# matvogel/P2P-Bridge

Measured on AMD Instinct MI355X. Metric: denoised points/sec (8192-pt patches, T=30), higher is better.
Workload: dtype f32; 1 GPU; PVDS_PUNet xyz-only, 8192-pt patches, T=30 bridge steps, batch 32 per GPU (BASELINE configs[1]); patches_per_gpu=32, points_per_patch=8192, bridge_steps=30, parallelism=patch-shard x1, process_group_world_size=1, hipgraph=True, weights=seeded random init (26.44 M params)

## Files before the change

p2p_bridge_amd/csrc/conv3d_farfield.hip:

```cpp
#include "conv3d_common.h"

static __global__ void far_value_kernel(int c, const float *__restrict__ base, const float *__restrict__ scale,
                                 const float *__restrict__ shift, int swish, float *__restrict__ a) {
  const int b = blockIdx.y, ch = blockIdx.x * 256 + threadIdx.x;
  if (ch >= c) return;
  a[(size_t)b * c + ch] = xf_apply(base[ch], scale[(size_t)b * c + ch], shift[(size_t)b * c + ch], swish);
}

static __global__ __launch_bounds__(256) void tap_sum_kernel(int cin, int cout, int nchunk, int cout_pad,
                                                      const float *__restrict__ wt, const float *__restrict__ a,
                                                      float *__restrict__ tsum) {
  const int tap = blockIdx.y, b = blockIdx.z;
  const int co = blockIdx.x * 256 + threadIdx.x;
  if (co >= cout) return;
  float acc = 0.0f;
  for (int ci = 0; ci < cin; ++ci) {
    const size_t idx = ((((size_t)tap * nchunk + (ci >> 3)) * 2 + (ci & 1)) * cout_pad + co) * 4 + ((ci & 7) >> 1);
    acc = __fmaf_rn(wt[idx], a[(size_t)b * cin + ci], acc);
  }
  tsum[((size_t)b * 27 + tap) * cout + co] = acc;
}

static __global__ __launch_bounds__(256) void class_bias_kernel(int cout, const float *__restrict__ tsum,
                                                         const float *__restrict__ bias, float *__restrict__ k_out) {
  const int cls = blockIdx.y, b = blockIdx.z;
  const int co = blockIdx.x * 256 + threadIdx.x;
  if (co >= cout) return;
  const int cd = cls / 9, ch = (cls / 3) % 3, cw = cls % 3;
  float acc = 0.0f;
  for (int tap = 0; tap < 27; ++tap) {
    const int kd = tap / 9, kh = (tap / 3) % 3, kw = tap % 3;
    if ((cd == 0 && kd == 0) || (cd == 2 && kd == 2) || (ch == 0 && kh == 0) || (ch == 2 && kh == 2) ||
        (cw == 0 && kw == 0) || (cw == 2 && kw == 2))
      continue;
    acc += tsum[((size_t)b * 27 + tap) * cout + co];
  }
  k_out[((size_t)b * 27 + cls) * cout + co] = acc + bias[co];
}

constexpr int FF_CO = 32;
static __global__ __launch_bounds__(1024) void far_field_kernel(int cin, int cout, int nchunk, int cout_pad,
                                                        const float *__restrict__ base, const float *__restrict__ scale,
                                                        const float *__restrict__ shift, int swish,
                                                        const float *__restrict__ wt, const float *__restrict__ bias,
                                                        float *__restrict__ a_out, float *__restrict__ k_out,
                                                        const float *__restrict__ part, int nslots, GnFinish fin) {
  extern __shared__ double ff_sm_d[];
  float *ff_sm = (float *)ff_sm_d;
  const int b = blockIdx.y, t = threadIdx.x, c = t & (FF_CO - 1), tap = t / FF_CO;
  const int co = blockIdx.x * FF_CO + c;
  float *a, *T;
  if (part != nullptr) {
    float *tsc = ff_sm, *tsh = ff_sm + cin;
    double *gl = ff_sm_d + (2 * cin + 1) / 2;
    GnFinish f = fin;
    if (blockIdx.x != 0) f.scale = f.shift = nullptr;
    gn_finish_sample<4>(cin, nslots, part, f, b, gl, tsc, tsh);
    a = (float *)gl, T = a + nchunk * 8;
    for (int ch = t; ch < cin; ch += 1024) {
      const float v = xf_apply(base[ch], tsc[ch], tsh[ch], swish);
      a[ch] = v;
      if (blockIdx.x == 0) a_out[(size_t)b * cin + ch] = v;
    }
  } else {
    a = ff_sm, T = ff_sm + nchunk * 8;
    for (int ch = t; ch < cin; ch += 1024) {
      const float v = xf_apply(base[ch], scale[(size_t)b * cin + ch], shift[(size_t)b * cin + ch], swish);
      a[ch] = v;
      if (blockIdx.x == 0) a_out[(size_t)b * cin + ch] = v;
    }
  }
  __syncthreads();
  if (tap < 27) {
    float acc = 0.0f;
    if (co < cout) {
      const float4 *w4 = (const float4 *)wt + ((size_t)tap * nchunk * 2) * cout_pad + co;
#pragma unroll 4
      for (int k8 = 0; k8 < nchunk; ++k8) {
        const float4 h0 = w4[(size_t)(2 * k8) * cout_pad], h1 = w4[(size_t)(2 * k8 + 1) * cout_pad];
        const float *av = a + k8 * 8;
        const int left = cin - k8 * 8;
        if (left > 0) acc = __fmaf_rn(h0.x, av[0], acc);
        if (left > 1) acc = __fmaf_rn(h1.x, av[1], acc);
        if (left > 2) acc = __fmaf_rn(h0.y, av[2], acc);
        if (left > 3) acc = __fmaf_rn(h1.y, av[3], acc);
        if (left > 4) acc = __fmaf_rn(h0.z, av[4], acc);
        if (left > 5) acc = __fmaf_rn(h1.z, av[5], acc);
        if (left > 6) acc = __fmaf_rn(h0.w, av[6], acc);
        if (left > 7) acc = __fmaf_rn(h1.w, av[7], acc);
      }
    }
    T[tap * FF_CO + c] = acc;
  }
  __syncthreads();
  if (co >= cout || tap >= 27) return;
  {
    const int cls = tap;
    const int cd = cls / 9, ch = (cls / 3) % 3, cw = cls % 3;
    float acc = 0.0f;
    for (int tp = 0; tp < 27; ++tp) {
      const int kd = tp / 9, kh = (tp / 3) % 3, kw = tp % 3;
      if ((cd == 0 && kd == 0) || (cd == 2 && kd == 2) || (ch == 0 && kh == 0) || (ch == 2 && kh == 2) ||
          (cw == 0 && kw == 0) || (cw == 2 && kw == 2))
        continue;
      acc += T[tp * FF_CO + c];
    }
    k_out[((size_t)b * 27 + cls) * cout + co] = acc + bias[co];
  }
}

static int far_field_launch(int b, int cin, int cout, const float *prev_bias, const float *in_scale, const float *in_shift,
                            int in_swish, const float *wt_packed, const float *bias, float *a, float *k_out, float *tap_ws,
                            const float *part, int nslots, const GnFinish &fin, hipStream_t s) {
  const int nchunk = (cin + CONV_CK - 1) / CONV_CK, cout_pad = (cout + 63) / 64 * 64;
  const size_t body = (size_t)(nchunk * 8 + 27 * FF_CO) * 4;
  const size_t lds = part ? (size_t)((2 * cin + 1) / 2) * 8 + (body > 32768 ? body : 32768) : body;
  if (lds <= 48 * 1024) {
    hipLaunchKernelGGL(far_field_kernel, dim3(cdiv(cout, FF_CO), b), dim3(1024), lds, s, cin, cout, nchunk, cout_pad, prev_bias,
                       in_scale, in_shift, in_swish, wt_packed, bias, a, k_out, part, nslots, fin);
    return p2pb_launch_status();
  }
  if (part) {
    const int e = p2pb_gn_affine_launch(b, cin, nslots, part, fin, s);
    if (e != 0) return e;
    in_scale = fin.scale, in_shift = fin.shift;
  }
  hipLaunchKernelGGL(far_value_kernel, dim3(cdiv(cin, 256), b), dim3(256), 0, s, cin, prev_bias, in_scale, in_shift,
                     in_swish, a);
  hipLaunchKernelGGL(tap_sum_kernel, dim3(cdiv(cout, 256), 27, b), dim3(256), 0, s, cin, cout, nchunk, cout_pad,
                     wt_packed, a, tap_ws);
  hipLaunchKernelGGL(class_bias_kernel, dim3(cdiv(cout, 256), 27, b), dim3(256), 0, s, cout, tap_ws, bias, k_out);
// ... 23 lines not shown
```

p2p_bridge_amd/csrc/neighbors.hip:

```cpp
#include "common.h"

template <int UNROLL>
__global__ __launch_bounds__(256) void ball_query_kernel(int n, int m, float r2, int u,
                                                         const float *__restrict__ centers,
                                                         const float *__restrict__ points, int *__restrict__ idx) {
  const int b = blockIdx.y;
  const int lane = lane_id();
  const int j = blockIdx.x * 4 + (threadIdx.x >> 6);
  if (j >= m) return;
  const float *p = points + (size_t)b * 3 * n;
  const float *ce = centers + (size_t)b * 3 * m;
  int *o = idx + ((size_t)b * m + j) * u;
  const float cx = ce[j], cy = ce[j + m], cz = ce[j + 2 * m];
  int cnt = 0, first = 0;
  for (int base = 0; base < n && cnt < u; base += 64 * UNROLL) {
    float px[UNROLL], py[UNROLL], pz[UNROLL];
#pragma unroll
    for (int q = 0; q < UNROLL; ++q) {
      const int k = base + q * 64 + lane;
      const bool ok = k < n;
      px[q] = ok ? p[k] : 0.0f;
      py[q] = ok ? p[k + n] : 0.0f;
      pz[q] = ok ? p[k + 2 * n] : 0.0f;
    }
// ... 119 lines not shown
  const int c0 = blockIdx.y * CC, c1 = min(c0 + CC, ct);
  for (int l = c0; l < c1; ++l) {
    float v;
    if (l < 3) v = coords[((size_t)b * 3 + l) * n + id] - centers[((size_t)b * 3 + l) * m + j];
    else v = feat[((size_t)b * c + (l - 3)) * n + id];
    out[((size_t)b * ct + l) * mu + q] = v;
  }
}

extern "C" int p2pb_group_concat(int b, int c, int n, int m, int u, const float *coords, const float *centers,
                                 const float *feat, const int *idx, float *out, void *stream) {
  if (b <= 0 || c < 0 || n <= 0 || m <= 0 || u <= 0) return P2PB_EINVAL;
  constexpr int CC = 8;
  hipLaunchKernelGGL(group_concat_kernel<CC>, dim3(cdiv((long)m * u, 256), cdiv(3 + c, CC), b), dim3(256), 0,
                     (hipStream_t)stream, c, n, m, u, coords, centers, feat, idx, out);
  return p2pb_launch_status();
}

__global__ __launch_bounds__(256) void nb_transpose_kernel(int c, int n, const float *__restrict__ in,
                                                           float *__restrict__ out) {
  __shared__ float t[32][33];
  const int b = blockIdx.z, n0 = blockIdx.x * 32, c0 = blockIdx.y * 32;
  const int tx = threadIdx.x & 31, ty = threadIdx.x >> 5;
  const float *src = in + (size_t)b * c * n;
  float *dst = out + (size_t)b * c * n;
#pragma unroll
  for (int k = 0; k < 4; ++k) {
    const int cc = c0 + ty + 8 * k, nn = n0 + tx;
    t[ty + 8 * k][tx] = (cc < c && nn < n) ? src[(size_t)cc * n + nn] : 0.0f;
  }
  __syncthreads();
#pragma unroll
  for (int k = 0; k < 4; ++k) {
    const int nn = n0 + ty + 8 * k, cc = c0 + tx;
    if (cc < c && nn < n) dst[(size_t)nn * c + cc] = t[tx][ty + 8 * k];
  }
}

__global__ __launch_bounds__(256) void group_sub_kernel(int c, int n, int m, int u, int nslots,
                                                        const float *__restrict__ zt, const float *__restrict__ cxt,
                                                        const int *__restrict__ idx, float *__restrict__ out,
                                                        float *__restrict__ stats) {
  __shared__ float tile[64][65];
  const int b = blockIdx.z, p0 = blockIdx.x * 64, t = threadIdx.x;
  const int lane = t & 63, wave = t >> 6;
  const int mu = m * u;
  const int qmine = p0 + wave * 16 + (lane & 15);
  const int id_mine = qmine < mu ? idx[(size_t)b * mu + qmine] : -1;
  const int cpl = c <= 32 ? 32 : 64, pps = 64 / cpl;
  const int sub = lane / cpl, chl = lane % cpl;
  {
    const int c0 = blockIdx.y * cpl;
    const int ch = c0 + chl;
#pragma unroll 4
    for (int it = 0; it < 16 / pps; ++it) {
      const int pl = wave * 16 + it * pps + sub;
      const int id = __shfl(id_mine, it * pps + sub);
      float v = 0.0f;
      if (id >= 0 && ch < c) {
        v = zt[((size_t)b * n + id) * c + ch];
        if (cxt) v -= cxt[((size_t)b * m + (p0 + pl) / u) * c + ch];
      }
      tile[chl][pl] = v;
    }
    __syncthreads();
    const int pt = lane;
    const int per = cpl / 4;
#pragma unroll
    for (int k = 0; k < 16; ++k) {
      const int cr = wave + 4 * k;
      const float v = tile[cr & 63][pt];
      if (k < per && c0 + cr < c) {
        if (out && p0 + pt < mu) out[((size_t)b * c + c0 + cr) * mu + p0 + pt] = v;
        const float s1 = halfwave_sum_to_last(v), s2 = halfwave_sum_to_last(v * v);
        if ((lane & 31) == 31) {
          float *p = stats + (((size_t)b * nslots + blockIdx.x * 2 + (lane >> 5)) * c + c0 + cr) * 2;
          p[0] = s1;
          p[1] = s2;
        }
      }
    }
    __syncthreads();
  }
}

#define GST_PW 128
template <int CPL>
__global__ __launch_bounds__(256) void group_stats_kernel(int c, int n, int m, int u, int nslots, const float *__restrict__ zt,
                                                          const float *__restrict__ cxt, const int *__restrict__ idx,
                                                          float *__restrict__ stats) {
  constexpr int PPS = 64 / CPL;
  const int b = blockIdx.z, lane = threadIdx.x & 63, wave = threadIdx.x >> 6;
  const int slot = blockIdx.x * 4 + wave;
  if (slot >= nslots) return;
  const int mu = m * u, p0 = slot * GST_PW;
  const int sub = lane / CPL, ch = blockIdx.y * CPL + lane % CPL;
  const int ia = p0 + lane < mu ? idx[(size_t)b * mu + p0 + lane] : -1;
  const int ib = p0 + 64 + lane < mu ? idx[(size_t)b * mu + p0 + 64 + lane] : -1;
  const float *zb = zt + (size_t)b * n * c + ch;
  const float *cb = cxt ? cxt + (size_t)b * m * c + ch : nullptr;
  float s1 = 0.0f, s2 = 0.0f;
  const bool chok = ch < c;
#pragma unroll 8
  for (int it = 0; it < GST_PW / PPS; ++it) {
    const int pl = it * PPS + sub;
    const int id = pl < 64 ? __shfl(ia, pl) : __shfl(ib, pl - 64);
    if (id >= 0 && chok) {
      float v = zb[(size_t)id * c];
      if (cb) v -= cb[(size_t)((p0 + pl) / u) * c];
      s1 += v;
      s2 += v * v;
    }
  }
  if (PPS == 2) {
    s1 += __shfl_xor(s1, 32);
    s2 += __shfl_xor(s2, 32);
  }
  if (chok && sub == 0) {
    float *q = stats + (((size_t)b * nslots + slot) * c + ch) * 2;
    q[0] = s1;
    q[1] = s2;
  }
}

extern "C" int p2pb_group_sub_stats_slots(int m, int u) { return (int)(((long)m * u + GST_PW - 1) / GST_PW); }
extern "C" int p2pb_group_sub_stats(int b, int c, int n, int m, int u, const float *zt, const float *cxt, const int *idx,
                                    float *stats_part, void *stream) {
  if (b <= 0 || c <= 0 || n <= 0 || m <= 0 || u <= 0 || !zt || !idx || !stats_part || (long)m * u > 0x7fffffffL) return P2PB_EINVAL;
  const int nslots = p2pb_group_sub_stats_slots(m, u);
  hipStream_t s = (hipStream_t)stream;
  if (c <= 32)
    hipLaunchKernelGGL(group_stats_kernel<32>, dim3(cdiv(nslots, 4), cdiv(c, 32), b), dim3(256), 0, s, c, n, m, u, nslots, zt, cxt, idx,
                       stats_part);
  else
    hipLaunchKernelGGL(group_stats_kernel<64>, dim3(cdiv(nslots, 4), cdiv(c, 64), b), dim3(256), 0, s, c, n, m, u, nslots, zt, cxt, idx,
                       stats_part);
  return p2pb_launch_status();
}

extern "C" size_t p2pb_group_sub_stats_floats(int b, int c, int m, int u) {
  return (size_t)b * (((size_t)m * u + 63) / 64 * 2) * c * 2;
}

extern "C" int p2pb_group_sub(int b, int c, int n, int m, int u, const float *z, const float *cx, const int *idx,
                              float *out, float *stats_part, float *ws, void *stream) {
  if (b <= 0 || c <= 0 || n <= 0 || m <= 0 || u <= 0 || !stats_part) return P2PB_EINVAL;
  hipStream_t s = (hipStream_t)stream;
  const float *zt = z, *cxt = cx;
  if (ws) {
    float *zw = ws, *cw = ws + (size_t)b * n * c;
    hipLaunchKernelGGL(nb_transpose_kernel, dim3(cdiv(n, 32), cdiv(c, 32), b), dim3(256), 0, s, c, n, z, zw);
    if (cx) hipLaunchKernelGGL(nb_transpose_kernel, dim3(cdiv(m, 32), cdiv(c, 32), b), dim3(256), 0, s, c, m, cx, cw);
    zt = zw;
    cxt = cx ? cw : nullptr;
  }
  const int nblk = (int)(((long)m * u + 63) / 64);
  hipLaunchKernelGGL(group_sub_kernel, dim3(nblk, cdiv(c, c <= 32 ? 32 : 64), b), dim3(256), 0, s, c, n, m, u, nblk * 2,
                     zt, cxt, idx, out, stats_part);
  return p2pb_launch_status();
}

__global__ __launch_bounds__(256) void gather_kernel(int c, int n, int m, const float *__restrict__ feat,
                                                     const int *__restrict__ idx, float *__restrict__ out) {
  const int b = blockIdx.z, l = blockIdx.y;
  const int j = blockIdx.x * 256 + threadIdx.x;
  if (j >= m) return;
  out[((size_t)b * c + l) * m + j] = feat[((size_t)b * c + l) * n + idx[(size_t)b * m + j]];
}

extern "C" int p2pb_gather_features_forward(int b, int c, int n, int m, const float *feat, const int *idx, float *out,
                                            void *stream) {
  if (b <= 0 || c <= 0 || n <= 0 || m <= 0) return P2PB_EINVAL;
  hipLaunchKernelGGL(gather_kernel, dim3(cdiv(m, 256), c, b), dim3(256), 0, (hipStream_t)stream, c, n, m, feat, idx,
                     out);
  return p2pb_launch_status();
}

#define NN_TILE 2048
__global__ __launch_bounds__(256) void three_nn_kernel(int n, int m, const float *__restrict__ points,
                                                       const float *__restrict__ centers, float *__restrict__ weights,
                                                       int *__restrict__ indices) {
  __shared__ float sc[3][NN_TILE];
  const int b = blockIdx.y;
  const int j = blockIdx.x * 256 + threadIdx.x;
  const float *p = points + (size_t)b * 3 * n;
  const float *ce = centers + (size_t)b * 3 * m;
  const bool ok = j < n;
  const float ux = ok ? p[j] : 0.0f, uy = ok ? p[j + n] : 0.0f, uz = ok ? p[j + 2 * n] : 0.0f;
  float best0 = INFINITY, best1 = INFINITY, best2 = INFINITY;
// ... 292 lines not shown
                                                 float *out, void *stream) {
  if (b <= 0 || c <= 0 || n <= 0 || m <= 0) return P2PB_EINVAL;
  hipStream_t s = (hipStream_t)stream;
  hipLaunchKernelGGL(three_nn_kernel, dim3(cdiv(n, 256), b), dim3(256), 0, s, n, m, points, centers, w, idx);
  constexpr int CC = 16;
  hipLaunchKernelGGL(three_interp_kernel<CC>, dim3(cdiv(n, 256), cdiv(c, CC), b), dim3(256), 0, s, c, m, n, cfeat,
                     idx, w, out);
  return p2pb_launch_status();
}

extern "C" int p2pb_three_nn(int b, int m, int n, const float *points, const float *centers, int *idx, float *w,
                             void *stream) {
  if (b <= 0 || n <= 0 || m <= 0) return P2PB_EINVAL;
  hipLaunchKernelGGL(three_nn_kernel, dim3(cdiv(n, 256), b), dim3(256), 0, (hipStream_t)stream, n, m, points, centers,
                     w, idx);
  return p2pb_launch_status();
}

extern "C" int p2pb_three_interpolate(int b, int c, int m, int n, const float *cfeat, const int *idx, const float *w,
                                      float *out, void *stream) {
  if (b <= 0 || c <= 0 || n <= 0 || m <= 0) return P2PB_EINVAL;
  constexpr int CC = 16;
  hipLaunchKernelGGL(three_interp_kernel<CC>, dim3(cdiv(n, 256), cdiv(c, CC), b), dim3(256), 0, (hipStream_t)stream, c,
                     m, n, cfeat, idx, w, out);
  return p2pb_launch_status();
}

__global__ __launch_bounds__(256) void three_interp_add_kernel(int c, int m, int n, int nslots,
                                                               const float *__restrict__ czt,
                                                               const int *__restrict__ indices,
                                                               const float *__restrict__ weights,
                                                               const float *__restrict__ add,
                                                               const float *__restrict__ bias, float *__restrict__ out,
                                                               float *__restrict__ stats) {
  __shared__ float tile[64][65];
  __shared__ int sid[64][3];
  __shared__ float sw[64][3];
  const int b = blockIdx.z, p0 = blockIdx.x * 64, t = threadIdx.x;
  const int lane = t & 63, wave = t >> 6;
  if (t < 64) {
    const int j = min(p0 + t, n - 1);
#pragma unroll
    for (int k = 0; k < 3; ++k) {
      sid[t][k] = indices[((size_t)b * 3 + k) * n + j];
      sw[t][k] = weights[((size_t)b * 3 + k) * n + j];
    }
  }
  __syncthreads();
  {
    const int c0 = blockIdx.y * 64;
    const int ch = c0 + lane;
    if (ch < c) {
      const float *f = czt + (size_t)b * m * c + ch;
#pragma unroll 4
      for (int pl = wave * 16; pl < wave * 16 + 16; ++pl)
        tile[lane][pl] = __fmaf_rn(f[(size_t)sid[pl][2] * c], sw[pl][2],
                                   __fmaf_rn(f[(size_t)sid[pl][1] * c], sw[pl][1], f[(size_t)sid[pl][0] * c] * sw[pl][0]));
    }
    __syncthreads();
    const int pt = lane;
    const bool pok = p0 + pt < n;
#pragma unroll
    for (int k = 0; k < 16; ++k) {
      const int cr = wave + 4 * k;
      if (c0 + cr < c) {
        float v = 0.0f;
        if (pok) {
          const size_t o = ((size_t)b * c + c0 + cr) * n + p0 + pt;
          v = tile[cr][pt];
          if (add) v += add[o];
          if (bias) v += bias[c0 + cr];
          out[o] = v;
        }
        const float s1 = halfwave_sum_to_last(v), s2 = halfwave_sum_to_last(v * v);
        if ((lane & 31) == 31) {
          float *p = stats + (((size_t)b * nslots + blockIdx.x * 2 + (lane >> 5)) * c + c0 + cr) * 2;
          p[0] = s1;
          p[1] = s2;
        }
      }
    }
    __syncthreads();
  }
}

extern "C" int p2pb_three_interpolate_add(int b, int c, int m, int n, const float *cz, const int *idx, const float *w,
                                          const float *add, const float *bias, float *out, float *stats_part,
                                          float *ws, void *stream) {
  if (b <= 0 || c <= 0 || n <= 0 || m <= 0 || !stats_part) return P2PB_EINVAL;
  hipStream_t s = (hipStream_t)stream;
  const float *czt = cz;
  if (ws) {
    hipLaunchKernelGGL(nb_transpose_kernel, dim3(cdiv(m, 32), cdiv(c, 32), b), dim3(256), 0, s, c, m, cz, ws);
    czt = ws;
  }
  const int nblk = (n + 63) / 64;
  hipLaunchKernelGGL(three_interp_add_kernel, dim3(nblk, cdiv(c, 64), b), dim3(256), 0, s, c, m, n, nblk * 2, czt, idx, w,
                     add, bias, out, stats_part);
  return p2pb_launch_status();
}
```

p2p_bridge_amd/csrc/pvconv_finish.hip:

```cpp
#include "common.h"

static __global__ __launch_bounds__(256) void gn_affine_kernel(int c, int groups, int nslots, double count_per_channel,
                                                        const float *__restrict__ part, const float *__restrict__ gamma,
                                                        const float *__restrict__ beta, const float *__restrict__ style,
                                                        int style_stride, float eps, float *__restrict__ scale,
                                                        float *__restrict__ shift, float *__restrict__ chmean,
                                                        float *__restrict__ mean_rstd) {
  __shared__ double lds[4 * 256];
  GnFinish f;
  f.gamma = gamma, f.beta = beta, f.style = style, f.scale = scale, f.shift = shift, f.chmean = chmean;
  f.count_per_channel = count_per_channel, f.style_stride = style_stride, f.groups = groups, f.eps = eps;
  gn_finish_group(c, nslots, part, f, blockIdx.y, blockIdx.x, lds, mean_rstd);
}

int p2pb_gn_affine_launch(int b, int c, int nslots, const float *part, const GnFinish &f, hipStream_t s) {
  hipLaunchKernelGGL(gn_affine_kernel, dim3(f.groups, b), dim3(256), 0, s, c, f.groups, nslots, f.count_per_channel, part, f.gamma,
                     f.beta, f.style, f.style_stride, f.eps, f.scale, f.shift, f.chmean, (float *)nullptr);
  return p2pb_launch_status();
}
extern "C" int p2pb_gn_affine_params_ex(int b, int c, int groups, int nslots, double count_per_channel,
                                        const float *part, const float *gamma, const float *beta, const float *style,
                                        int style_stride, float eps, float *scale, float *shift, float *chmean,
                                        float *mean_rstd, void *stream) {
  if (b <= 0 || c <= 0 || nslots <= 0 || !gn_shape_ok(c, groups, style, style_stride)) return P2PB_EINVAL;
  hipLaunchKernelGGL(gn_affine_kernel, dim3(groups, b), dim3(256), 0, (hipStream_t)stream, c, groups, nslots,
                     count_per_channel, part, gamma, beta, style, style_stride, eps, scale, shift, chmean, mean_rstd);
  return p2pb_launch_status();
}

extern "C" int p2pb_gn_affine_params(int b, int c, int groups, int nslots, double count_per_channel,
                                     const float *part, const float *gamma, const float *beta, const float *style,
                                     int style_stride, float eps, float *scale, float *shift, float *chmean,
                                     void *stream) {
  return p2pb_gn_affine_params_ex(b, c, groups, nslots, count_per_channel, part, gamma, beta, style, style_stride, eps,
                                  scale, shift, chmean, nullptr, stream);
}

__device__ __forceinline__ void se_hidden(int c, int hidden, const float *__restrict__ w1, const float *mean, float *hid) {
  const int lane = threadIdx.x & 63, wave = threadIdx.x >> 6, nw = blockDim.x >> 6;
  for (int h = wave; h < hidden; h += nw) {
    float acc = 0.0f;
    for (int i = lane; i < c; i += 64) acc = __fmaf_rn(w1[(size_t)h * c + i], mean[i], acc);
#pragma unroll
    for (int d = 32; d >= 1; d >>= 1) acc += __shfl_xor(acc, d);
    if (lane == 0) hid[h] = fmaxf(acc, 0.0f);
  }
}


static __global__ __launch_bounds__(256) void se_gate_affine_kernel(int c, int hidden, const float *__restrict__ chmean,
                                                             const float *__restrict__ w1, const float *__restrict__ w2,
                                                             const float *__restrict__ scale,
                                                             const float *__restrict__ shift, float *__restrict__ aff_a,
                                                             float *__restrict__ aff_b) {
  extern __shared__ float se_sm[];
  float *mean = se_sm, *hid = se_sm + c;
  const int b = blockIdx.x, t = threadIdx.x;
  for (int i = t; i < c; i += 256) mean[i] = chmean[(size_t)b * c + i];
  __syncthreads();
  se_hidden(c, hidden, w1, mean, hid);
  __syncthreads();
  for (int i = t; i < c; i += 256) {
    float acc = 0.0f;
    for (int h = 0; h < hidden; ++h) acc = __fmaf_rn(w2[(size_t)i * hidden + h], hid[h], acc);
    const float gate = 1.0f / (1.0f + expf(-acc));
    aff_a[(size_t)b * c + i] = scale[(size_t)b * c + i] * gate;
    aff_b[(size_t)b * c + i] = shift[(size_t)b * c + i] * gate;
  }
}

static __global__ __launch_bounds__(1024) void pvconv_tail_kernel(int c, int hidden, const float *__restrict__ part2, int nslots2,
                                                           GnFinish f2, const float *__restrict__ w1, const float *__restrict__ w2,
                                                           float *__restrict__ aff_a, float *__restrict__ aff_b,
                                                           int cp, const float *__restrict__ partp, int nslotsp, GnFinish fp) {
  extern __shared__ double pt_sm[];
  const int b = blockIdx.y, t = threadIdx.x;
  if (blockIdx.x == 1) {
    gn_finish_sample<4>(cp, nslotsp, partp, fp, b, pt_sm);
    return;
  }
  float *sc = (float *)(pt_sm + 4096), *sh = sc + c, *mean = sh + c, *hid = mean + c;
  gn_finish_sample<4>(c, nslots2, part2, f2, b, pt_sm, sc, sh, mean);
  if (hidden <= 0) {
    for (int i = t; i < c; i += 1024) {
      aff_a[(size_t)b * c + i] = sc[i];
      aff_b[(size_t)b * c + i] = sh[i];
    }
    return;
  }
  se_hidden(c, hidden, w1, mean, hid);
  __syncthreads();
  for (int i = t; i < c; i += 1024) {
    float acc = 0.0f;
    for (int h = 0; h < hidden; ++h) acc = __fmaf_rn(w2[(size_t)i * hidden + h], hid[h], acc);
    const float gate = 1.0f / (1.0f + expf(-acc));
// ... 34 lines not shown
```

p2p_bridge_amd/csrc/voxelize.hip:

```cpp
#include "common.h"

__global__ __launch_bounds__(1024) void voxel_coords_kernel(int n, int r, int normalize, float eps,
                                                            const float *__restrict__ coords,
                                                            float *__restrict__ norm, int *__restrict__ vox) {
  __shared__ double part[3][256];
  __shared__ float smax[1024];
  const int t = threadIdx.x;
  const float *c = coords + (size_t)blockIdx.x * 3 * n;
  float *o = norm + (size_t)blockIdx.x * 3 * n;
  int *v = vox + (size_t)blockIdx.x * 3 * n;
  if (t < 256) {
    double s0 = 0.0, s1 = 0.0, s2 = 0.0;
    for (int k0 = t; k0 < n; k0 += 8 * 256) {
      float x0[8], x1[8], x2[8];
#pragma unroll
      for (int u = 0; u < 8; ++u) {
        const int k = k0 + u * 256;
        const bool ok = k < n;
        x0[u] = ok ? c[k] : 0.0f;
        x1[u] = ok ? c[n + k] : 0.0f;
        x2[u] = ok ? c[2 * n + k] : 0.0f;
      }
#pragma unroll
      for (int u = 0; u < 8; ++u)
// ... 287 lines not shown
#pragma unroll
        for (int i = 0; i < 4; ++i)
          if (i < nch) acc[i] += fq[i] * div;
      }
    }
  }
  float *o = out + ((size_t)b * r3 + v) * c + ch;
  if (ALIGNED) {
    *(vox_f32x4 *)o = vox_f32x4{acc[0], acc[1], acc[2], acc[3]};
  } else {
#pragma unroll
    for (int i = 0; i < 4; ++i)
      if (i < nch) o[i] = acc[i];
  }
}

__global__ __launch_bounds__(256) void vox_gather_cl_occ_kernel(int c, int n, int r3, const int *__restrict__ cnt,
                                                                const int *__restrict__ cur,
                                                                const int *__restrict__ occ,
                                                                const int *__restrict__ nocc,
                                                                const int *__restrict__ slist,
                                                                const float *__restrict__ feat_t,
                                                                float *__restrict__ out) {
  const int b = blockIdx.y;
  const size_t total = (size_t)nocc[b] * c;
  for (size_t e = (size_t)blockIdx.x * 256 + threadIdx.x; e < total; e += (size_t)gridDim.x * 256) {
    const int k = (int)(e / c), ch = (int)(e % c);
    const int v = occ[(size_t)b * n + k];
    const int cn = cnt[(size_t)b * r3 + v];
    const int *seg = slist + (size_t)b * n + (cur[(size_t)b * r3 + v] - cn);
    const float div = (float)(1.0 / (double)(float)cn);
    const float *f = feat_t + (size_t)b * n * c + ch;
    float acc = 0.0f;
    for (int q = 0; q < cn; ++q) acc += f[(size_t)seg[q] * c] * div;
    out[((size_t)b * r3 + v) * c + ch] = acc;
  }
}

template <bool ALIGNED>
__global__ __launch_bounds__(256) void vox_gather_cl_split_kernel(int c, int nchunk, int n, int r3,
                                                                  const int *__restrict__ cnt, const int *__restrict__ cur,
                                                                  const int *__restrict__ slist,
                                                                  const float *__restrict__ feat_t, u32x4 *__restrict__ out) {
  const int b = blockIdx.y, ng = nchunk * 2;
  const size_t e = (size_t)blockIdx.x * 256 + threadIdx.x;
  if (e >= (size_t)r3 * ng) return;
  const int v = (int)(e / ng), g = (int)(e % ng), ch = g * 8;
  const int cn = cnt[(size_t)b * r3 + v];
  float acc[8] = {0.0f, 0.0f, 0.0f, 0.0f, 0.0f, 0.0f, 0.0f, 0.0f};
  if (cn > 0 && ch < c) {
    const int *seg = slist + (size_t)b * n + (cur[(size_t)b * r3 + v] - cn);
    const float div = (float)(1.0 / (double)(float)cn);
    const float *f = feat_t + (size_t)b * n * c + ch;
    for (int q = 0; q < cn; ++q) {
      const float *fq = f + (size_t)seg[q] * c;
      if (ALIGNED) {
#pragma unroll
        for (int h = 0; h < 2; ++h)
          if (ch + 4 * h < c) {
            const vox_f32x4 x = *(const vox_f32x4 *)(fq + 4 * h);
#pragma unroll
            for (int i = 0; i < 4; ++i) acc[4 * h + i] += x[i] * div;
          }
      } else {
#pragma unroll
        for (int i = 0; i < 8; ++i)
          if (ch + i < c) acc[i] += fq[i] * div;
      }
    }
  }
  u32x4 p0, p1;
#pragma unroll
  for (int i = 0; i < 4; ++i) {
    unsigned a0, a1, a2;
    split_pair<SPLIT_F16X3>(acc[2 * i], acc[2 * i + 1], a0, a1, a2);
    p0[i] = a0;
    p1[i] = a1;
  }
  u32x4 *dst = out + (((size_t)b * r3 + v) * nchunk + (g >> 1)) * 4 + (g & 1);
  dst[0] = p0;
  dst[2] = p1;
}

template <bool ALIGNED>
__global__ __launch_bounds__(256) void vox_gather_cl_occ_split_kernel(int c, int nchunk, int n, int r3,
                                                                      const int *__restrict__ cnt, const int *__restrict__ cur,
                                                                      const int *__restrict__ occ, const int *__restrict__ nocc,
                                                                      const int *__restrict__ slist,
                                                                      const float *__restrict__ feat_t, u32x4 *__restrict__ out) {
  const int b = blockIdx.y, ng = nchunk * 2;
  const size_t total = (size_t)nocc[b] * ng;
  for (size_t e = (size_t)blockIdx.x * 256 + threadIdx.x; e < total; e += (size_t)gridDim.x * 256) {
    const int k = (int)(e / ng), g = (int)(e % ng), ch = g * 8;
    const int v = occ[(size_t)b * n + k];
    const int cn = cnt[(size_t)b * r3 + v];
    const int *seg = slist + (size_t)b * n + (cur[(size_t)b * r3 + v] - cn);
    const float div = (float)(1.0 / (double)(float)cn);
    const float *f = feat_t + (size_t)b * n * c + ch;
    float acc[8] = {0.0f, 0.0f, 0.0f, 0.0f, 0.0f, 0.0f, 0.0f, 0.0f};
    for (int q0 = 0; q0 < cn; q0 += 4) {
      int id[4];
#pragma unroll
      for (int u = 0; u < 4; ++u) id[u] = seg[min(q0 + u, cn - 1)];
      float x[4][8];
#pragma unroll
      for (int u = 0; u < 4; ++u) {
        const float *fq = f + (size_t)id[u] * c;
        if (ALIGNED) {
#pragma unroll
          for (int h = 0; h < 2; ++h) {
            vox_f32x4 y = vox_f32x4{0.0f, 0.0f, 0.0f, 0.0f};
            if (ch + 4 * h < c) y = *(const vox_f32x4 *)(fq + 4 * h);
#pragma unroll
            for (int i = 0; i < 4; ++i) x[u][4 * h + i] = y[i];
          }
        } else {
#pragma unroll
          for (int i = 0; i < 8; ++i) x[u][i] = ch + i < c ? fq[i] : 0.0f;
        }
      }
#pragma unroll
// ... 206 lines not shown
extern "C" int p2pb_trilinear_devoxelize_forward(int b, int c, int n, int r, int is_training, const float *coords,
                                                 const float *feat, int *inds, float *wgts, float *outs,
                                                 void *stream) {
  if (b <= 0 || c <= 0 || n <= 0 || r <= 0) return P2PB_EINVAL;
  if (is_training && (!inds || !wgts)) return P2PB_EINVAL;
  constexpr int CC = 16;
  hipLaunchKernelGGL((devox_kernel<CC, false>), dim3(cdiv(n, 256), cdiv(c, CC), b), dim3(256), 0, (hipStream_t)stream,
                     c, n, r, is_training, coords, feat, (const float *)nullptr, (const float *)nullptr, inds, wgts,
                     outs);
  return p2pb_launch_status();
}

extern "C" int p2pb_trilinear_devoxelize_affine(int b, int c, int n, int r, const float *coords, const float *feat,
                                                const float *aff_a, const float *aff_b, float *outs, void *stream) {
  if (b <= 0 || c <= 0 || n <= 0 || r <= 0 || !aff_a || !aff_b) return P2PB_EINVAL;
  constexpr int CC = 16;
  hipLaunchKernelGGL((devox_kernel<CC, true>), dim3(cdiv(n, 256), cdiv(c, CC), b), dim3(256), 0, (hipStream_t)stream,
                     c, n, r, 0, coords, feat, aff_a, aff_b, (int *)nullptr, (float *)nullptr, outs);
  return p2pb_launch_status();
}

__global__ __launch_bounds__(256) void devox_cl_kernel(int c, int n, int r, const float *__restrict__ coords,
                                                       const float *__restrict__ grid, const float *__restrict__ aff_a,
                                                       const float *__restrict__ aff_b, const float *__restrict__ add,
                                                       const float *__restrict__ add_scale,
                                                       const float *__restrict__ add_shift, float *__restrict__ outs) {
  __shared__ float tile[64][65];
  __shared__ __attribute__((aligned(16))) int sidx[64][8];
  __shared__ __attribute__((aligned(16))) float sw[64][8];
  const int b = blockIdx.z, p0 = blockIdx.x * 64, t = threadIdx.x;
  const int lane = t & 63, wave = t >> 6;
  const int r3 = r * r * r;
  if (lane < 16) {
    const int tt = wave * 16 + lane;
    const int i = min(p0 + tt, n - 1);
    const float *co = coords + (size_t)b * 3 * n;
    const Corners k = devox_corners(co[i], co[i + n], co[i + 2 * n], r);
    typedef int i32x4 __attribute__((ext_vector_type(4)));
    typedef float f32x4 __attribute__((ext_vector_type(4)));
#define DV_LDS __attribute__((address_space(3)))
    *(volatile DV_LDS i32x4 *)&sidx[tt][0] = i32x4{k.idx[0], k.idx[1], k.idx[2], k.idx[3]};
    *(volatile DV_LDS i32x4 *)&sidx[tt][4] = i32x4{k.idx[4], k.idx[5], k.idx[6], k.idx[7]};
    *(volatile DV_LDS f32x4 *)&sw[tt][0] = f32x4{k.w[0], k.w[1], k.w[2], k.w[3]};
    *(volatile DV_LDS f32x4 *)&sw[tt][4] = f32x4{k.w[4], k.w[5], k.w[6], k.w[7]};
#undef DV_LDS
  }
  __syncthreads();
  const float *g = grid + (size_t)b * r3 * c;
  {
    const int c0 = blockIdx.y * 64;
    const int ch = c0 + lane;
    if (ch < c) {
      const float a = aff_a ? aff_a[(size_t)b * c + ch] : 1.0f, bb = aff_b ? aff_b[(size_t)b * c + ch] : 0.0f;
#pragma unroll 2
      for (int pl = wave * 16; pl < wave * 16 + 16; ++pl) {
        float fv[8];
#pragma unroll
        for (int q = 0; q < 8; ++q) fv[q] = g[(size_t)sidx[pl][q] * c + ch];
        if (aff_a) {
#pragma unroll
          for (int q = 0; q < 8; ++q) fv[q] = fv[q] * a + bb;
        }
        float acc = sw[pl][0] * fv[0];
#pragma unroll
        for (int q = 1; q < 8; ++q) acc = __fmaf_rn(sw[pl][q], fv[q], acc);
        tile[lane][pl] = acc;
      }
    }
    __syncthreads();
    const int pt = t & 63;
    if (p0 + pt < n) {
#pragma unroll
      for (int k = 0; k < 16; ++k) {
        const int cr = (t >> 6) + 4 * k;
        if (c0 + cr < c) {
          const size_t o = ((size_t)b * c + c0 + cr) * n + p0 + pt;
          float v = tile[cr][pt];
          if (add) {
            const float z = add[o] * add_scale[(size_t)b * c + c0 + cr] + add_shift[(size_t)b * c + c0 + cr];
            v = z * __builtin_amdgcn_rcpf(1.0f + __builtin_amdgcn_exp2f(z * -1.44269504088896340736f)) + v;
          }
          outs[o] = v;
        }
      }
    }
    __syncthreads();
  }
}

__global__ __launch_bounds__(256) void devox_cl4_kernel(int c, int n, int r, const float *__restrict__ coords,
                                                        const float *__restrict__ grid, const float *__restrict__ aff_a,
                                                        const float *__restrict__ aff_b, const float *__restrict__ add,
                                                        const float *__restrict__ add_scale,
                                                        const float *__restrict__ add_shift, float *__restrict__ outs) {
  __shared__ float tile[64][65];
  __shared__ __attribute__((aligned(16))) int sidx[64][8];
  __shared__ __attribute__((aligned(16))) float sw[64][8];
  typedef int i32x4 __attribute__((ext_vector_type(4)));
  typedef float f32x4 __attribute__((ext_vector_type(4)));
  const int b = blockIdx.z, p0 = blockIdx.x * 64, t = threadIdx.x;
  const int lane = t & 63, wave = t >> 6;
  const int r3 = r * r * r;
  if (lane < 16) {
    const int tt = wave * 16 + lane;
    const int i = min(p0 + tt, n - 1);
    const float *co = coords + (size_t)b * 3 * n;
    const Corners k = devox_corners(co[i], co[i + n], co[i + 2 * n], r);
#define DV_LDS __attribute__((address_space(3)))
    *(volatile DV_LDS i32x4 *)&sidx[tt][0] = i32x4{k.idx[0], k.idx[1], k.idx[2], k.idx[3]};
    *(volatile DV_LDS i32x4 *)&sidx[tt][4] = i32x4{k.idx[4], k.idx[5], k.idx[6], k.idx[7]};
    *(volatile DV_LDS f32x4 *)&sw[tt][0] = f32x4{k.w[0], k.w[1], k.w[2], k.w[3]};
    *(volatile DV_LDS f32x4 *)&sw[tt][4] = f32x4{k.w[4], k.w[5], k.w[6], k.w[7]};
#undef DV_LDS
  }
  __syncthreads();
  const float *g = grid + (size_t)b * r3 * c;
  const int c0 = blockIdx.y * 64;
  {
    const int cq = lane & 15, ps = lane >> 4;
    const int ch4 = c0 + 4 * cq;
    f32x4 a4 = {1.0f, 1.0f, 1.0f, 1.0f}, b4 = {0.0f, 0.0f, 0.0f, 0.0f};
    if (aff_a) {
      a4 = *(const f32x4 *)(aff_a + (size_t)b * c + ch4);
      b4 = *(const f32x4 *)(aff_b + (size_t)b * c + ch4);
    }
#pragma unroll 2
    for (int it = 0; it < 4; ++it) {
      const int pl = wave * 16 + it * 4 + ps;
      f32x4 fv[8];
#pragma unroll
      for (int q = 0; q < 8; ++q) fv[q] = *(const f32x4 *)(g + (size_t)sidx[pl][q] * c + ch4);
      if (aff_a) {
#pragma unroll
        for (int q = 0; q < 8; ++q)
#pragma unroll
          for (int i = 0; i < 4; ++i) fv[q][i] = fv[q][i] * a4[i] + b4[i];
      }
#pragma unroll
      for (int i = 0; i < 4; ++i) {
        float acc = sw[pl][0] * fv[0][i];
#pragma unroll
        for (int q = 1; q < 8; ++q) acc = __fmaf_rn(sw[pl][q], fv[q][i], acc);
        tile[4 * cq + i][pl] = acc;
      }
    }
  }
  __syncthreads();
  const int pt = t & 63;
  if (p0 + pt < n) {
#pragma unroll
    for (int k = 0; k < 16; ++k) {
      const int cr = (t >> 6) + 4 * k;
      const size_t o = ((size_t)b * c + c0 + cr) * n + p0 + pt;
      float v = tile[cr][pt];
      if (add) {
        const float z = add[o] * add_scale[(size_t)b * c + c0 + cr] + add_shift[(size_t)b * c + c0 + cr];
        v = z * __builtin_amdgcn_rcpf(1.0f + __builtin_amdgcn_exp2f(z * -1.44269504088896340736f)) + v;
      }
      outs[o] = v;
    }
  }
}

extern "C" int p2pb_trilinear_devoxelize_cl_affine(int b, int c, int n, int r, const float *coords, const float *grid,
                                                   const float *aff_a, const float *aff_b, const float *add,
                                                   const float *add_scale, const float *add_shift, float *outs,
                                                   void *stream) {
  if (b <= 0 || c <= 0 || n <= 0 || r <= 0 || ((aff_a == nullptr) != (aff_b == nullptr))) return P2PB_EINVAL;
  if (add && (!add_scale || !add_shift)) return P2PB_EINVAL;
  static const long wide = p2pb_experiment_long("devox_cl4", 1);
  if (wide && c % 64 == 0 && (((size_t)grid | (size_t)aff_a | (size_t)aff_b) & 15) == 0)
    hipLaunchKernelGGL(devox_cl4_kernel, dim3(cdiv(n, 64), c / 64, b), dim3(256), 0, (hipStream_t)stream, c, n, r, coords, grid,
                       aff_a, aff_b, add, add_scale, add_shift, outs);
  else
    hipLaunchKernelGGL(devox_cl_kernel, dim3(cdiv(n, 64), cdiv(c, 64), b), dim3(256), 0, (hipStream_t)stream, c, n, r, coords, grid,
                       aff_a, aff_b, add, add_scale, add_shift, outs);
  return p2pb_launch_status();
}
```

Baseline: 1.197 million points/s.

## Batch independent gather loads ahead of use across several memory-bound kernels

Several gather and reduction loops (far-field tap sums, group gather and group stats, the SE hidden matvec, voxel averaging, and trilinear devoxelization) are rewritten to issue a batch of independent global loads into registers before consuming them, using clamped indices and selects instead of guarded loads. Epilogue operands (residual add, scale and shift, bias) are prefetched before the barrier so their latency overlaps with the tile computation. Group stats also gains a compile-time flag for the centroid-subtract path. The aim is more memory-level parallelism in latency-bound gathers, paid for with higher register pressure, possible occupancy loss, and redundant clamped loads for out-of-range elements.

```diff
diff --git a/p2p_bridge_amd/csrc/conv3d_farfield.hip b/p2p_bridge_amd/csrc/conv3d_farfield.hip
--- a/p2p_bridge_amd/csrc/conv3d_farfield.hip
+++ b/p2p_bridge_amd/csrc/conv3d_farfield.hip
@@ -75,8 +75,26 @@
     float acc = 0.0f;
     if (co < cout) {
       const float4 *w4 = (const float4 *)wt + ((size_t)tap * nchunk * 2) * cout_pad + co;
-#pragma unroll 4
-      for (int k8 = 0; k8 < nchunk; ++k8) {
+      int k8 = 0;
+      for (; k8 + 4 <= cin / 8; k8 += 4) {
+        float4 h[8];
+#pragma unroll
+        for (int q = 0; q < 8; ++q) h[q] = w4[(size_t)(2 * k8 + q) * cout_pad];
+#pragma unroll
+        for (int q = 0; q < 4; ++q) {
+          const float4 h0 = h[2 * q], h1 = h[2 * q + 1];
+          const float *av = a + (k8 + q) * 8;
+          acc = __fmaf_rn(h0.x, av[0], acc);
+          acc = __fmaf_rn(h1.x, av[1], acc);
+          acc = __fmaf_rn(h0.y, av[2], acc);
+          acc = __fmaf_rn(h1.y, av[3], acc);
+          acc = __fmaf_rn(h0.z, av[4], acc);
+          acc = __fmaf_rn(h1.z, av[5], acc);
+          acc = __fmaf_rn(h0.w, av[6], acc);
+          acc = __fmaf_rn(h1.w, av[7], acc);
+        }
+      }
+      for (; k8 < nchunk; ++k8) {
         const float4 h0 = w4[(size_t)(2 * k8) * cout_pad], h1 = w4[(size_t)(2 * k8 + 1) * cout_pad];
         const float *av = a + k8 * 8;
         const int left = cin - k8 * 8;
diff --git a/p2p_bridge_amd/csrc/neighbors.hip b/p2p_bridge_amd/csrc/neighbors.hip
--- a/p2p_bridge_amd/csrc/neighbors.hip
+++ b/p2p_bridge_amd/csrc/neighbors.hip
@@ -195,16 +195,31 @@
   {
     const int c0 = blockIdx.y * cpl;
     const int ch = c0 + chl;
-#pragma unroll 4
-    for (int it = 0; it < 16 / pps; ++it) {
-      const int pl = wave * 16 + it * pps + sub;
-      const int id = __shfl(id_mine, it * pps + sub);
-      float v = 0.0f;
-      if (id >= 0 && ch < c) {
-        v = zt[((size_t)b * n + id) * c + ch];
-        if (cxt) v -= cxt[((size_t)b * m + (p0 + pl) / u) * c + ch];
-      }
-      tile[chl][pl] = v;
+    const float *zb = zt + (size_t)b * n * c + min(ch, c - 1);
+    const float *cb = cxt ? cxt + (size_t)b * m * c + min(ch, c - 1) : nullptr;
+    int cj = (p0 + wave * 16 + sub) / u, cr = (p0 + wave * 16 + sub) - cj * u;
+    for (int it0 = 0; it0 < 16 / pps; it0 += 8) {
+      int id[8];
+      float zv[8], cv[8];
+#pragma unroll
+      for (int k = 0; k < 8; ++k) {
+        id[k] = __shfl(id_mine, (it0 + k) * pps + sub);
+        zv[k] = zb[(size_t)max(id[k], 0) * c];
+        cv[k] = cb ? cb[(size_t)min(cj, m - 1) * c] : 0.0f;
+#pragma unroll
+        for (int q = 0; q < 2; ++q) {
+          const bool wrap = q < pps && cr + 1 == u;
+          cr = wrap ? 0 : (q < pps ? cr + 1 : cr);
+          cj += wrap ? 1 : 0;
+        }
+      }
+#pragma unroll
+      for (int k = 0; k < 8; ++k) {
+        const int pl = wave * 16 + (it0 + k) * pps + sub;
+        float v = zv[k];
+        if (cb) v -= cv[k];
+        tile[chl][pl] = (id[k] >= 0 && ch < c) ? v : 0.0f;
+      }
     }
     __syncthreads();
     const int pt = lane;
@@ -228,7 +243,8 @@
 }
 
 #define GST_PW 128
-template <int CPL>
+#define GST_NB 16
+template <int CPL, bool CX>
 __global__ __launch_bounds__(256) void group_stats_kernel(int c, int n, int m, int u, int nslots, const float *__restrict__ zt,
                                                           const float *__restrict__ cxt, const int *__restrict__ idx,
                                                           float *__restrict__ stats) {
@@ -240,19 +256,40 @@
   const int sub = lane / CPL, ch = blockIdx.y * CPL + lane % CPL;
   const int ia = p0 + lane < mu ? idx[(size_t)b * mu + p0 + lane] : -1;
   const int ib = p0 + 64 + lane < mu ? idx[(size_t)b * mu + p0 + 64 + lane] : -1;
-  const float *zb = zt + (size_t)b * n * c + ch;
-  const float *cb = cxt ? cxt + (size_t)b * m * c + ch : nullptr;
+  const bool chok = ch < c;
+  const float *zb = zt + (size_t)b * n * c + min(ch, c - 1);
+  const float *cb = CX ? cxt + (size_t)b * m * c + min(ch, c - 1) : nullptr;
+  int cj = (p0 + sub) / u, cr = (p0 + sub) - cj * u;
   float s1 = 0.0f, s2 = 0.0f;
-  const bool chok = ch < c;
-#pragma unroll 8
-  for (int it = 0; it < GST_PW / PPS; ++it) {
-    const int pl = it * PPS + sub;
-    const int id = pl < 64 ? __shfl(ia, pl) : __shfl(ib, pl - 64);
-    if (id >= 0 && chok) {
-      float v = zb[(size_t)id * c];
-      if (cb) v -= cb[(size_t)((p0 + pl) / u) * c];
-      s1 += v;
-      s2 += v * v;
+#pragma unroll 1
+  for (int pb = 0; pb < GST_PW; pb += GST_NB * PPS) {
+    const int src = pb < 64 ? ia : ib;
+    int id[GST_NB];
+    float zv[GST_NB], cv[GST_NB];
+#pragma unroll
+    for (int k = 0; k < GST_NB; ++k) {
+      const int l = (pb & 63) + k * PPS;
+      id[k] = __builtin_amdgcn_readlane(src, l);
+      if (PPS == 2) id[k] = sub ? __builtin_amdgcn_readlane(src, l + 1) : id[k];
+      zv[k] = zb[(size_t)max(id[k], 0) * c];
+      if (CX) {
+        cv[k] = cb[(size_t)min(cj, m - 1) * c];
+#pragma unroll
+        for (int q = 0; q < PPS; ++q) {
+          const bool wrap = cr + 1 == u;
+          cr = wrap ? 0 : cr + 1;
+          cj += wrap ? 1 : 0;
+        }
+      }
+    }
+#pragma unroll
+    for (int k = 0; k < GST_NB; ++k) {
+      float v = zv[k];
+      if (CX) v -= cv[k];
+      const bool ok = id[k] >= 0 && chok;
+      const float t1 = s1 + v, t2 = s2 + v * v;
+      s1 = ok ? t1 : s1;
+      s2 = ok ? t2 : s2;
     }
   }
   if (PPS == 2) {
@@ -264,6 +301,14 @@
     q[0] = s1;
     q[1] = s2;
   }
+}
+
+template <int CPL>
+static void group_stats_launch(int b, int c, int n, int m, int u, int nslots, const float *zt, const float *cxt, const int *idx,
+                               float *stats_part, hipStream_t s) {
+  const dim3 grid(cdiv(nslots, 4), cdiv(c, CPL), b);
+  if (cxt) hipLaunchKernelGGL((group_stats_kernel<CPL, true>), grid, dim3(256), 0, s, c, n, m, u, nslots, zt, cxt, idx, stats_part);
+  else hipLaunchKernelGGL((group_stats_kernel<CPL, false>), grid, dim3(256), 0, s, c, n, m, u, nslots, zt, cxt, idx, stats_part);
 }
 
 extern "C" int p2pb_group_sub_stats_slots(int m, int u) { return (int)(((long)m * u + GST_PW - 1) / GST_PW); }
@@ -272,12 +317,8 @@
   if (b <= 0 || c <= 0 || n <= 0 || m <= 0 || u <= 0 || !zt || !idx || !stats_part || (long)m * u > 0x7fffffffL) return P2PB_EINVAL;
   const int nslots = p2pb_group_sub_stats_slots(m, u);
   hipStream_t s = (hipStream_t)stream;
-  if (c <= 32)
-    hipLaunchKernelGGL(group_stats_kernel<32>, dim3(cdiv(nslots, 4), cdiv(c, 32), b), dim3(256), 0, s, c, n, m, u, nslots, zt, cxt, idx,
-                       stats_part);
-  else
-    hipLaunchKernelGGL(group_stats_kernel<64>, dim3(cdiv(nslots, 4), cdiv(c, 64), b), dim3(256), 0, s, c, n, m, u, nslots, zt, cxt, idx,
-                       stats_part);
+  if (c <= 32) group_stats_launch<32>(b, c, n, m, u, nslots, zt, cxt, idx, stats_part, s);
+  else group_stats_launch<64>(b, c, n, m, u, nslots, zt, cxt, idx, stats_part, s);
   return p2pb_launch_status();
 }
 
@@ -676,26 +717,38 @@
     const int ch = c0 + lane;
     if (ch < c) {
       const float *f = czt + (size_t)b * m * c + ch;
-#pragma unroll 4
-      for (int pl = wave * 16; pl < wave * 16 + 16; ++pl)
-        tile[lane][pl] = __fmaf_rn(f[(size_t)sid[pl][2] * c], sw[pl][2],
-                                   __fmaf_rn(f[(size_t)sid[pl][1] * c], sw[pl][1], f[(size_t)sid[pl][0] * c] * sw[pl][0]));
-    }
-    __syncthreads();
+      for (int pl0 = wave * 16; pl0 < wave * 16 + 16; pl0 += 8) {
+        float g[8][3];
+#pragma unroll
+        for (int k = 0; k < 8; ++k)
+#pragma unroll
+          for (int q = 0; q < 3; ++q) g[k][q] = f[(size_t)sid[pl0 + k][q] * c];
+#pragma unroll
+        for (int k = 0; k < 8; ++k)
+          tile[lane][pl0 + k] = __fmaf_rn(g[k][2], sw[pl0 + k][2], __fmaf_rn(g[k][1], sw[pl0 + k][1], g[k][0] * sw[pl0 + k][0]));
+      }
+    }
     const int pt = lane;
     const bool pok = p0 + pt < n;
+    float av[16], bv[16];
+    if (add) {
+#pragma unroll
+      for (int k = 0; k < 16; ++k) av[k] = add[((size_t)b * c + min(c0 + wave + 4 * k, c - 1)) * n + min(p0 + pt, n - 1)];
+    }
+    if (bias) {
+#pragma unroll
+      for (int k = 0; k < 16; ++k) bv[k] = bias[min(c0 + wave + 4 * k, c - 1)];
+    }
+    __syncthreads();
 #pragma unroll
     for (int k = 0; k < 16; ++k) {
       const int cr = wave + 4 * k;
       if (c0 + cr < c) {
-        float v = 0.0f;
-        if (pok) {
-          const size_t o = ((size_t)b * c + c0 + cr) * n + p0 + pt;
-          v = tile[cr][pt];
-          if (add) v += add[o];
-          if (bias) v += bias[c0 + cr];
-          out[o] = v;
-        }
+        float v = tile[cr][pt];
+        if (add) v += av[k];
+        if (bias) v += bv[k];
+        v = pok ? v : 0.0f;
+        if (pok) out[((size_t)b * c + c0 + cr) * n + p0 + pt] = v;
         const float s1 = halfwave_sum_to_last(v), s2 = halfwave_sum_to_last(v * v);
         if ((lane & 31) == 31) {
           float *p = stats + (((size_t)b * nslots + blockIdx.x * 2 + (lane >> 5)) * c + c0 + cr) * 2;
diff --git a/p2p_bridge_amd/csrc/pvconv_finish.hip b/p2p_bridge_amd/csrc/pvconv_finish.hip
--- a/p2p_bridge_amd/csrc/pvconv_finish.hip
+++ b/p2p_bridge_amd/csrc/pvconv_finish.hip
@@ -40,7 +40,17 @@
   const int lane = threadIdx.x & 63, wave = threadIdx.x >> 6, nw = blockDim.x >> 6;
   for (int h = wave; h < hidden; h += nw) {
     float acc = 0.0f;
-    for (int i = lane; i < c; i += 64) acc = __fmaf_rn(w1[(size_t)h * c + i], mean[i], acc);
+    for (int i0 = lane; i0 < c; i0 += 64 * 8) {
+      float wv[8];
+#pragma unroll
+      for (int q = 0; q < 8; ++q) wv[q] = w1[(size_t)h * c + min(i0 + 64 * q, c - 1)];
+#pragma unroll
+      for (int q = 0; q < 8; ++q) {
+        const int i = i0 + 64 * q;
+        const float t = __fmaf_rn(wv[q], mean[min(i, c - 1)], acc);
+        acc = i < c ? t : acc;
+      }
+    }
 #pragma unroll
     for (int d = 32; d >= 1; d >>= 1) acc += __shfl_xor(acc, d);
     if (lane == 0) hid[h] = fmaxf(acc, 0.0f);
diff --git a/p2p_bridge_amd/csrc/voxelize.hip b/p2p_bridge_amd/csrc/voxelize.hip
--- a/p2p_bridge_amd/csrc/voxelize.hip
+++ b/p2p_bridge_amd/csrc/voxelize.hip
@@ -363,21 +363,34 @@
     const int *seg = slist + (size_t)b * n + (cur[(size_t)b * r3 + v] - cn);
     const float div = (float)(1.0 / (double)(float)cn);
     const float *f = feat_t + (size_t)b * n * c + ch;
-    for (int q = 0; q < cn; ++q) {
-      const float *fq = f + (size_t)seg[q] * c;
-      if (ALIGNED) {
-#pragma unroll
-        for (int h = 0; h < 2; ++h)
-          if (ch + 4 * h < c) {
-            const vox_f32x4 x = *(const vox_f32x4 *)(fq + 4 * h);
-#pragma unroll
-            for (int i = 0; i < 4; ++i) acc[4 * h + i] += x[i] * div;
+    for (int q0 = 0; q0 < cn; q0 += 4) {
+      int id[4];
+#pragma unroll
+      for (int u = 0; u < 4; ++u) id[u] = seg[min(q0 + u, cn - 1)];
+      float x[4][8];
+#pragma unroll
+      for (int u = 0; u < 4; ++u) {
+        const float *fq = f + (size_t)id[u] * c;
+        if (ALIGNED) {
+#pragma unroll
+          for (int h = 0; h < 2; ++h) {
+            vox_f32x4 y = vox_f32x4{0.0f, 0.0f, 0.0f, 0.0f};
+            if (ch + 4 * h < c) y = *(const vox_f32x4 *)(fq + 4 * h);
+#pragma unroll
+            for (int i = 0; i < 4; ++i) x[u][4 * h + i] = y[i];
           }
-      } else {
-#pragma unroll
-        for (int i = 0; i < 8; ++i)
-          if (ch + i < c) acc[i] += fq[i] * div;
-      }
+        } else {
+#pragma unroll
+          for (int i = 0; i < 8; ++i) x[u][i] = ch + i < c ? fq[i] : 0.0f;
+        }
+      }
+#pragma unroll
+      for (int u = 0; u < 4; ++u)
+        if (q0 + u < cn) {
+#pragma unroll
+          for (int i = 0; i < 8; ++i)
+            if (ch + (ALIGNED ? i & 4 : i) < c) acc[i] += x[u][i] * div;
+        }
     }
   }
   u32x4 p0, p1;
@@ -690,23 +703,38 @@
     const int ch = c0 + lane;
     if (ch < c) {
       const float a = aff_a ? aff_a[(size_t)b * c + ch] : 1.0f, bb = aff_b ? aff_b[(size_t)b * c + ch] : 0.0f;
-#pragma unroll 2
-      for (int pl = wave * 16; pl < wave * 16 + 16; ++pl) {
-        float fv[8];
-#pragma unroll
-        for (int q = 0; q < 8; ++q) fv[q] = g[(size_t)sidx[pl][q] * c + ch];
-        if (aff_a) {
-#pragma unroll
-          for (int q = 0; q < 8; ++q) fv[q] = fv[q] * a + bb;
+      for (int pl0 = wave * 16; pl0 < wave * 16 + 16; pl0 += 2) {
+        float fv[2][8];
+#pragma unroll
+        for (int u = 0; u < 2; ++u)
+#pragma unroll
+          for (int q = 0; q < 8; ++q) fv[u][q] = g[(size_t)sidx[pl0 + u][q] * c + ch];
+#pragma unroll
+        for (int u = 0; u < 2; ++u) {
+          const int pl = pl0 + u;
+          if (aff_a) {
+#pragma unroll
+            for (int q = 0; q < 8; ++q) fv[u][q] = fv[u][q] * a + bb;
+          }
+          float acc = sw[pl][0] * fv[u][0];
+#pragma unroll
+          for (int q = 1; q < 8; ++q) acc = __fmaf_rn(sw[pl][q], fv[u][q], acc);
+          tile[lane][pl] = acc;
         }
-        float acc = sw[pl][0] * fv[0];
-#pragma unroll
-        for (int q = 1; q < 8; ++q) acc = __fmaf_rn(sw[pl][q], fv[q], acc);
-        tile[lane][pl] = acc;
+      }
+    }
+    const int pt = t & 63;
+    float hv[16], hsc[16], hsh[16];
+    if (add) {
+#pragma unroll
+      for (int k = 0; k < 16; ++k) {
+        const size_t row = (size_t)b * c + min(c0 + (t >> 6) + 4 * k, c - 1);
+        hv[k] = add[row * n + min(p0 + pt, n - 1)];
+        hsc[k] = add_scale[row];
+        hsh[k] = add_shift[row];
       }
     }
     __syncthreads();
-    const int pt = t & 63;
     if (p0 + pt < n) {
 #pragma unroll
       for (int k = 0; k < 16; ++k) {
@@ -715,7 +743,7 @@
           const size_t o = ((size_t)b * c + c0 + cr) * n + p0 + pt;
           float v = tile[cr][pt];
           if (add) {
-            const float z = add[o] * add_scale[(size_t)b * c + c0 + cr] + add_shift[(size_t)b * c + c0 + cr];
+            const float z = hv[k] * hsc[k] + hsh[k];
             v = z * __builtin_amdgcn_rcpf(1.0f + __builtin_amdgcn_exp2f(z * -1.44269504088896340736f)) + v;
           }
           outs[o] = v;
@@ -783,8 +811,18 @@
       }
     }
   }
+  const int pt = t & 63;
+  float hv[16], hsc[16], hsh[16];
+  if (add) {
+#pragma unroll
+    for (int k = 0; k < 16; ++k) {
+      const size_t row = (size_t)b * c + c0 + (t >> 6) + 4 * k;
+      hv[k] = add[row * n + min(p0 + pt, n - 1)];
+      hsc[k] = add_scale[row];
+      hsh[k] = add_shift[row];
+    }
+  }
   __syncthreads();
-  const int pt = t & 63;
   if (p0 + pt < n) {
 #pragma unroll
     for (int k = 0; k < 16; ++k) {
@@ -792,7 +830,7 @@
       const size_t o = ((size_t)b * c + c0 + cr) * n + p0 + pt;
       float v = tile[cr][pt];
       if (add) {
-        const float z = add[o] * add_scale[(size_t)b * c + c0 + cr] + add_shift[(size_t)b * c + c0 + cr];
+        const float z = hv[k] * hsc[k] + hsh[k];
         v = z * __builtin_amdgcn_rcpf(1.0f + __builtin_amdgcn_exp2f(z * -1.44269504088896340736f)) + v;
       }
       outs[o] = v;
```

After: 1.222 million points/s (median of 6 runs). 1.02x the previous value.
